# nianticlabs/implicit-depth

Measured on AMD Instinct MI355X. Metric: frames/sec (BDModel.forward hot path, 512x384, 64 planes, 8-frame tuple = 1 current + 7 source views; third-party backbones excluded), higher is better.
Workload: dtype f32

## Files before the change

### implicit-depth_amd/csrc/feature_volume.hip

```cpp
#include <stdlib.h>

#include "idh_common.h"
#include "split_f16.h"

namespace {

using namespace idh_f16;

constexpr int kC = 16;
constexpr int kHid = 128;
constexpr int kNS = 8;
constexpr int kMaxK = 8;

constexpr int kWsHom = 0, kWsT = 192, kWsInvK = 256, kWsBias = 272;
static_assert(kWsT == 12 * IDH_MAX_SOURCE_VIEWS && kWsInvK == kWsT + 4 * IDH_MAX_SOURCE_VIEWS && kWsBias + kHid <= 400, "workspace layout");
constexpr int kWsStrideReal = 400;

__device__ __forceinline__ float lrelu01(float x) {
#ifdef IDH_ABL_FV2_NOACT
    return x;
#endif
    return __builtin_elementwise_maximum(x, x * 0.01f);
}
__device__ __forceinline__ float lrelu01_sel(float x) { return x >= 0.f ? x : x * 0.01f; }

__device__ __forceinline__ float fv_depth_plane(int i, int D, float dmin, float dmax) {
    float ramp = 0.f;
    if (D > 1) {
        const float step = 1.0f / (float)(D - 1);
        ramp = (i < D / 2) ? step * (float)i : 1.0f - step * (float)(D - 1 - i);
    }
    return expf(logf(dmin) + logf(dmax / dmin) * ramp);
}

__global__ void fv_setup_k(const float *__restrict__ src_K, const float *__restrict__ src_E,
                           const float *__restrict__ src_poses, const float *__restrict__ cur_invK,
                           const float *__restrict__ w1_pose, const float *__restrict__ b1, int K,
                           float *__restrict__ ws) {
    const int b = blockIdx.x, t = threadIdx.x;
    float *o = ws + (size_t)b * kWsStrideReal;
    __shared__ float s_pd[3 * IDH_MAX_SOURCE_VIEWS];
    if (t < K) {
        const float *Km = src_K + (size_t)(b * K + t) * 16, *Em = src_E + (size_t)(b * K + t) * 16;
        const float *iK = cur_invK + (size_t)b * 16, *Pm = src_poses + (size_t)(b * K + t) * 16;
        float P[3][4];
        for (int i = 0; i < 3; ++i)
            for (int j = 0; j < 4; ++j) {
                float s = 0.f;
                for (int m = 0; m < 4; ++m) s = fmaf(Km[i * 4 + m], Em[m * 4 + j], s);
                P[i][j] = s;
            }
        float *h = o + kWsHom + 12 * t;
        for (int i = 0; i < 3; ++i) {
            for (int j = 0; j < 3; ++j) {
                float s = 0.f;
                for (int m = 0; m < 3; ++m) s = fmaf(P[i][m], iK[m * 4 + j], s);
                h[i * 3 + j] = s;
            }
            h[9 + i] = P[i][3];
        }
        o[kWsT + 4 * t + 0] = Pm[3]; o[kWsT + 4 * t + 1] = Pm[7]; o[kWsT + 4 * t + 2] = Pm[11]; o[kWsT + 4 * t + 3] = 0.f;
        const float tr = Pm[0] + Pm[5] + Pm[10];
        const float rm = sqrtf(2.f * (1.f - fminf(3.f, tr) / 3.f));
        const float tm = sqrtf(Pm[3] * Pm[3] + Pm[7] * Pm[7] + Pm[11] * Pm[11]);
        s_pd[t] = sqrtf(tm * tm + rm * rm);
        s_pd[K + t] = rm;
        s_pd[2 * K + t] = tm;
    }
    if (t < 9) o[kWsInvK + t] = cur_invK[(size_t)b * 16 + (t / 3) * 4 + (t % 3)];
    __syncthreads();
    if (t < kHid) {
        float s = b1[t];
        for (int j = 0; j < 3 * K; ++j) s = fmaf(w1_pose[(size_t)t * 3 * K + j], s_pd[j], s);
        o[kWsBias + t] = s;
    }
}

struct FvArgs {
    const float *cur;
    const float *src;
    const float *ws;
    const float *w1v;
    const float *w1p;
    const float *w2;
    const float *vecs;
    float *vol;
    unsigned char *mask;
    int vol_cs;
    int B, K, H, W, D;
    int tiles_per_img;
    int DP, G;
    int J, MB;
    float dmin, dmax;
    long long cur_bs, src_bs;
    const float *planes;
    long long planes_sb, planes_sd;
    int planes_sp;
};

__device__ __forceinline__ float fv_plane(const FvArgs &a, int b, int p, int d) {
    return a.planes ? a.planes[(size_t)b * a.planes_sb + (size_t)d * a.planes_sd + (size_t)p * a.planes_sp]
                    : fv_depth_plane(d, a.D, a.dmin, a.dmax);
}

template <int KT>
__global__ __launch_bounds__(512) void fv_mlp_k(const FvArgs a) {
    extern __shared__ __attribute__((aligned(16))) unsigned char smem_raw[];
    f32x4 *sW1 = reinterpret_cast<f32x4 *>(smem_raw);
    f32x4 *sW2 = sW1 + (a.K + 4) * kNS * 64;
    {
        const f32x4 *g1 = reinterpret_cast<const f32x4 *>(a.w1v);
        const f32x4 *g2 = reinterpret_cast<const f32x4 *>(a.w2);
        const int n1 = (a.K + 4) * kNS * 64, n2 = kNS * kNS * 64;
        for (int i = threadIdx.x; i < n1; i += 512) sW1[i] = g1[i];
        for (int i = threadIdx.x; i < n2; i += 512) sW2[i] = g2[i];
    }
    __syncthreads();
    const float *s_b2 = a.vecs, *s_w3 = a.vecs + kHid;
    const float b3 = a.vecs[2 * kHid];

    const int lane = threadIdx.x & 63;
    const int wave = __builtin_amdgcn_readfirstlane(threadIdx.x >> 6);
    const int ln = lane & 15, q = lane >> 4;
    const int N = a.H * a.W;
    const int K = KT > 0 ? KT : a.K;
    const float Wf = (float)a.W, Hf = (float)a.H;
    const long long ntasks = (long long)a.B * a.tiles_per_img * a.G;

    for (long long task = (long long)idh_xcd_remap(blockIdx.x, gridDim.x) * 8 + wave; task < ntasks; task += (long long)gridDim.x * 8) {
        const int g = __builtin_amdgcn_readfirstlane((int)(task % a.G));
        const int tile = __builtin_amdgcn_readfirstlane((int)((task / a.G) % a.tiles_per_img));
        const int b = __builtin_amdgcn_readfirstlane((int)(task / ((long long)a.G * a.tiles_per_img)));
        const int p_raw = tile * 16 + ln;
        const bool live = p_raw < N;
        const int p = live ? p_raw : N - 1;
        const int py = p / a.W, px = p - py * a.W;
        const float pxf = (float)px + 0.5f, pyf = (float)py + 0.5f;
        const float *pb = a.ws + (size_t)b * kWsStrideReal;

        const f32x4 cur4 = *reinterpret_cast<const f32x4 *>(a.cur + (size_t)b * a.cur_bs + (size_t)p * kC + 4 * q);
        const float *iK = pb + kWsInvK;
        const float rx = fmaf(iK[0], pxf, fmaf(iK[1], pyf, iK[2]));
        const float ry = fmaf(iK[3], pxf, fmaf(iK[4], pyf, iK[5]));
        const float rz = fmaf(iK[6], pxf, fmaf(iK[7], pyf, iK[8]));

        f32x4 pre[kNS];
#pragma unroll
        for (int i = 0; i < kNS; ++i) pre[i] = *reinterpret_cast<const f32x4 *>(pb + kWsBias + 16 * i + 4 * q);
        const int d0 = g * a.DP, d1 = min(a.D, d0 + a.DP);
        if (d0 >= d1) continue;
        const float rn = fmaxf(sqrtf(rx * rx + ry * ry + rz * rz), 1e-12f);
        const float crx = rx / rn, cry = ry / rn, crz = rz / rn;
        {
            const f32x4 rayB = (q == 0) ? (f32x4){crx, cry, crz, 0.f} : (f32x4){0.f, 0.f, 0.f, 0.f};
            const f32x4 *w1p = reinterpret_cast<const f32x4 *>(a.w1p);
#pragma unroll
            for (int i = 0; i < kNS; ++i) {
                const f32x4 A0 = w1p[(0 * kNS + i) * 64 + lane];
                const f32x4 A1 = w1p[(1 * kNS + i) * 64 + lane];
#pragma unroll
                for (int kk = 0; kk < 4; ++kk) pre[i] = __builtin_amdgcn_mfma_f32_16x16x4f32(A0[kk], cur4[kk], pre[i], 0, 0, 0);
#pragma unroll
                for (int kk = 0; kk < 4; ++kk) pre[i] = __builtin_amdgcn_mfma_f32_16x16x4f32(A1[kk], rayB[kk], pre[i], 0, 0, 0);
            }
        }

        const int ov[2] = {min(q, K - 1), min(q + 4, K - 1)};
        float oq[2][3], oh[2][3];
#pragma unroll
        for (int jv = 0; jv < 2; ++jv) {
            const float *hm = pb + kWsHom + 12 * ov[jv];
            oq[jv][0] = fmaf(hm[0], pxf, fmaf(hm[1], pyf, hm[2]));
            oq[jv][1] = fmaf(hm[3], pxf, fmaf(hm[4], pyf, hm[5]));
            oq[jv][2] = fmaf(hm[6], pxf, fmaf(hm[7], pyf, hm[8]));
            oh[jv][0] = hm[9]; oh[jv][1] = hm[10]; oh[jv][2] = hm[11];
        }
        const __amdgpu_buffer_rsrc_t rsS = __builtin_amdgcn_make_buffer_rsrc(const_cast<float *>(a.src + (size_t)b * a.src_bs), 0, K * N * kC * 4, 0x00020000);
        const int bp0 = 4 * ln;

        f32x4 ob = (f32x4){0.f, 0.f, 0.f, 0.f};
        const bool vec_ok = ((d0 & 3) == 0) && ((a.vol_cs & 3) == 0) && ((reinterpret_cast<uintptr_t>(a.vol) & 15) == 0);
        struct Own { int pk; float w00, w01, w10, w11, z; };
        struct Pro { Own own[2]; float depth, m3, m4, m5, m6, m10, m11, m12, m13; };
        struct Tap { f32x4 t00, t01, t10, t11; };
        struct Wts { float w00, w01, w10, w11; };
        float oc[2][3];
#pragma unroll
        for (int jv = 0; jv < 2; ++jv) {
            const float *t = pb + kWsT + 4 * ov[jv];
            oc[jv][0] = t[0]; oc[jv][1] = t[1]; oc[jv][2] = t[2];
        }
        auto prologue = [&](int d) {
            Pro P;
            const float depth = fv_plane(a, b, p, d);
            P.depth = depth;
#pragma unroll
            for (int jv = 0; jv < 2; ++jv) {
#ifdef IDH_ABL_FV2_NOPRO
                P.own[jv].pk = p; P.own[jv].w00 = P.own[jv].w01 = P.own[jv].w10 = P.own[jv].w11 = depth; P.own[jv].z = depth;
                continue;
#endif
                const float cx = fmaf(depth, oq[jv][0], oh[jv][0]);
                const float cy = fmaf(depth, oq[jv][1], oh[jv][1]);
                const float cz = fmaf(depth, oq[jv][2], oh[jv][2]);
                const float z = fmaxf(cz, 1e-5f);
                float r = __builtin_amdgcn_rcpf(z);
                r = r * fmaf(-z, r, 2.0f);
                const float su = cx * r, sv = cy * r;
                const float sx = fminf(fmaxf(su - 0.5f, -1.0f), Wf);
                const float sy = fminf(fmaxf(sv - 0.5f, -1.0f), Hf);
                const float x0f = floorf(sx), y0f = floorf(sy);
                const float fx = sx - x0f, fy = sy - y0f;
                const int x0 = (int)x0f, y0 = (int)y0f;
                const float wx0 = (x0 >= 0 && x0 < a.W) ? 1.0f - fx : 0.f;
                const float wx1 = (x0 + 1 < a.W) ? fx : 0.f;
                const float wy0 = (y0 >= 0 && y0 < a.H) ? 1.0f - fy : 0.f;
                const float wy1 = (y0 + 1 < a.H) ? fy : 0.f;
                const int xa0 = min(max(x0, 0), a.W - 1), xa1 = min(x0 + 1, a.W - 1);
                const int ya0 = min(max(y0, 0), a.H - 1), ya1 = min(y0 + 1, a.H - 1);
                P.own[jv].pk = (ya0 * a.W + xa0) | ((xa1 - xa0) << 30) | ((ya1 - ya0) << 31);
                P.own[jv].w00 = wx0 * wy0; P.own[jv].w01 = wx1 * wy0; P.own[jv].w10 = wx0 * wy1; P.own[jv].w11 = wx1 * wy1;
                P.own[jv].z = z;
            }
            const float Xx = depth * rx, Xy = depth * ry, Xz = depth * rz;
            auto ray = [&](int jv, float &ang, float &e0, float &e1, float &e2) {
                const float ax = Xx - oc[jv][0], ay = Xy - oc[jv][1], az = Xz - oc[jv][2];
                const float n2 = fmaf(az, az, fmaf(ay, ay, ax * ax));
                float in = __builtin_amdgcn_rsqf(fmaxf(n2, 1e-24f));
                in = in * fmaf(-0.5f * n2 * in, in, 1.5f);
                e0 = ax * in; e1 = ay * in; e2 = az * in;
                ang = fmaf(crz, e2, fmaf(cry, e1, crx * e0));
            };
#ifdef IDH_ABL_FV2_NORAY
            P.m3 = P.m4 = P.m5 = P.m6 = P.m10 = P.m11 = P.m12 = P.m13 = depth;
            return P;
#endif
            ray(0, P.m3, P.m4, P.m5, P.m6);
            ray(1, P.m10, P.m11, P.m12, P.m13);
            return P;
        };
        auto issue = [&](const Pro &P, int k) {
            const int pk = __builtin_amdgcn_ds_bpermute(bp0 + 64 * (k & 3), P.own[k >> 2].pk);
            const int o00 = ((pk & 0x3fffffff) << 6) + 16 * q;
            const int o01 = o00 + (((pk >> 30) & 1) << 6);
            const int ystep = (int)((unsigned)pk >> 31) * (a.W * 64);
            Tap t;
#ifdef IDH_ABL_FV2_NOTAPS
            t.t00 = t.t01 = t.t10 = t.t11 = (f32x4){1.f + (float)o00, 2.f + (float)o01, 3.f + (float)ystep, 4.f};
            return t;
#endif
            const int so = __builtin_amdgcn_readfirstlane(k * N * (kC * 4));
            t.t00 = __builtin_bit_cast(f32x4, __builtin_amdgcn_raw_buffer_load_b128(rsS, o00, so, 0));
            t.t01 = __builtin_bit_cast(f32x4, __builtin_amdgcn_raw_buffer_load_b128(rsS, o01, so, 0));
            t.t10 = __builtin_bit_cast(f32x4, __builtin_amdgcn_raw_buffer_load_b128(rsS, o00 + ystep, so, 0));
            t.t11 = __builtin_bit_cast(f32x4, __builtin_amdgcn_raw_buffer_load_b128(rsS, o01 + ystep, so, 0));
            return t;
        };
        auto weights = [&](const Pro &P, int k) {
            const Own &o = P.own[k >> 2];
            auto bperm = [&](float v) -> float { return __builtin_bit_cast(float, __builtin_amdgcn_ds_bpermute(bp0 + 64 * (k & 3), __builtin_bit_cast(int, v))); };
            Wts w;
            w.w00 = bperm(o.w00); w.w01 = bperm(o.w01); w.w10 = bperm(o.w10); w.w11 = bperm(o.w11);
            return w;
        };
        Pro P = prologue(d0);
        Tap cur = issue(P, 0);
        Wts wc = weights(P, 0);
#pragma unroll 1
        for (int d = d0; d < d1; ++d) {
            const float depth = P.depth;
            f32x4 acc1[kNS];
#pragma unroll
            for (int i = 0; i < kNS; ++i) acc1[i] = pre[i];
            float m2 = 0.f, m9 = 0.f;
            const float m1 = q < K ? P.own[0].z : 0.f;
            float m8 = q + 4 < K ? P.own[1].z : 0.f;
            __builtin_amdgcn_s_setprio(2);
            constexpr int KU = KT > 0 ? KT : kMaxK;
#pragma unroll
            for (int k = 0; k < KU; ++k) {
                if (KT == 0 && k >= K) break;
                const int kn = (KT > 0) ? (k + 1 < KT ? k + 1 : k) : k + 1;
                Tap nxt = cur;
                Wts wn = wc;
                if (kn != k && kn < KU) { nxt = issue(P, kn); wn = weights(P, kn); }
                f32x4 wv;
#ifdef IDH_ABL_FV2_NOBLEND
                wv = cur.t00 + cur.t11;
                float part = wc.w00 + wc.w11 + cur.t01[0] + cur.t10[0];
#else
#pragma unroll
                for (int e = 0; e < 4; ++e)
                    wv[e] = fmaf(wc.w11, cur.t11[e], fmaf(wc.w10, cur.t10[e], fmaf(wc.w01, cur.t01[e], wc.w00 * cur.t00[e])));
                float part = wv[0] * cur4[0];
                part = fmaf(wv[1], cur4[1], part); part = fmaf(wv[2], cur4[2], part); part = fmaf(wv[3], cur4[3], part);
                part += __shfl_xor(part, 16, 64);
                part += __shfl_xor(part, 32, 64);
#endif
                const float dotv = part;
                const bool s0 = (k == q), s1 = (k == q + 4);
                m2 = s0 ? dotv : m2;
                m9 = s1 ? dotv : m9;
#pragma unroll
                for (int i = 0; i < kNS; ++i) {
#ifdef IDH_ABL_FV2_NOLDSA
                    const f32x4 A = (f32x4){1.f, 2.f, 3.f, 4.f} * (float)(i + 1);
#else
                    const f32x4 A = sW1[(k * kNS + i) * 64 + lane];
#endif
#pragma unroll
                    for (int kk = 0; kk < 4; ++kk) acc1[i] = __builtin_amdgcn_mfma_f32_16x16x4f32(A[kk], wv[kk], acc1[i], 0, 0, 0);
                }
                if constexpr (KT > 0) {
#pragma unroll
                    for (int r = 0; r < 16; ++r) {
                        __builtin_amdgcn_sched_group_barrier(0x008, 2, 0);
#ifndef IDH_ABL_FV_VALU_PER_GROUP
#define IDH_ABL_FV_VALU_PER_GROUP 3
#endif
                        __builtin_amdgcn_sched_group_barrier(0x002, IDH_ABL_FV_VALU_PER_GROUP, 0);
                    }
                }
                cur = nxt;
                wc = wn;
            }
            const float m3 = P.m3, m4 = P.m4, m5 = P.m5, m6 = P.m6, m10 = P.m10, m11 = P.m11, m12 = P.m12, m13 = P.m13;
            const bool depth_in_q3 = K < 8;
            if (depth_in_q3 && q == 3) m8 = depth;
            const f32x4 mb[4] = {(f32x4){m1, m2, m3, m4}, (f32x4){m5, m6, m8, m9}, (f32x4){m10, m11, m12, m13}, (f32x4){depth, 0.f, 0.f, 0.f}};
#pragma unroll
            for (int c = 0; c < 3; ++c) {
#pragma unroll
                for (int i = 0; i < kNS; ++i) {
                    const f32x4 A = sW1[((K + c) * kNS + i) * 64 + lane];
#pragma unroll
                    for (int kk = 0; kk < 4; ++kk) acc1[i] = __builtin_amdgcn_mfma_f32_16x16x4f32(A[kk], mb[c][kk], acc1[i], 0, 0, 0);
                }
            }
            if (!depth_in_q3) {
#pragma unroll
                for (int i = 0; i < kNS; ++i) {
                    const float A0 = reinterpret_cast<const float *>(&sW1[((K + 3) * kNS + i) * 64 + lane])[0];
                    acc1[i] = __builtin_amdgcn_mfma_f32_16x16x4f32(A0, mb[3][0], acc1[i], 0, 0, 0);
                }
            }
            f32x4 acc2[kNS];
            Pro Pn;
            Tap curn;
            Wts wcn;
#pragma unroll
            for (int i = 0; i < kNS; ++i) {
#pragma unroll
                for (int r = 0; r < 4; ++r) acc1[i][r] = lrelu01(acc1[i][r]);
                acc2[i] = *reinterpret_cast<const f32x4 *>(s_b2 + 16 * i + 4 * q);
            }
            __builtin_amdgcn_s_setprio(0);
#pragma unroll
            for (int c = 0; c < kNS; ++c) {
#pragma unroll
                for (int i = 0; i < kNS; ++i) {
#ifdef IDH_ABL_FV2_NOLDSA
                    const f32x4 A = (f32x4){1.f, 2.f, 3.f, 4.f} * (float)(i + 1);
#else
                    const f32x4 A = sW2[(c * kNS + i) * 64 + lane];
#endif
#pragma unroll
                    for (int kk = 0; kk < 4; ++kk) acc2[i] = __builtin_amdgcn_mfma_f32_16x16x4f32(A[kk], acc1[c][kk], acc2[i], 0, 0, 0);
                }
                if (c == (KT > 0 ? 0 : 1)) {
                    Pn = prologue(min(d + 1, d1 - 1));
                    curn = issue(Pn, 0);
                    wcn = weights(Pn, 0);
                }
                if constexpr (KT == 0) __builtin_amdgcn_sched_barrier(0);
            }
            float s = 0.f;
#ifdef IDH_ABL_FV2_NOL3
#pragma unroll
            for (int i = 0; i < kNS; ++i) s += acc2[i][0];
#else
#pragma unroll
            for (int i = 0; i < kNS; ++i) {
                const f32x4 w3 = *reinterpret_cast<const f32x4 *>(s_w3 + 16 * i + 4 * q);
#pragma unroll
                for (int r = 0; r < 4; ++r) s = fmaf(w3[r], lrelu01(acc2[i][r]), s);
            }
            s += __shfl_xor(s, 16, 64);
            s += __shfl_xor(s, 32, 64);
#endif
            const float val = s + b3;
            if (a.vol_cs > 0) {
                const int e = (d - d0) & 3;
                ob[0] = e == 0 ? val : ob[0]; ob[1] = e == 1 ? val : ob[1]; ob[2] = e == 2 ? val : ob[2]; ob[3] = e == 3 ? val : ob[3];
                if (q == 0 && live && (e == 3 || d == d1 - 1)) {
                    float *o = a.vol + ((size_t)b * N + p) * a.vol_cs + (d - e);
                    if (e == 3 && vec_ok) *reinterpret_cast<f32x4 *>(o) = ob;
                    else { o[0] = ob[0]; if (e >= 1) o[1] = ob[1]; if (e >= 2) o[2] = ob[2]; if (e >= 3) o[3] = ob[3]; }
                }
            } else if (q == 0 && live) {
                a.vol[((size_t)b * a.D + d) * N + p] = val;
            }
            if (a.mask != nullptr && d == a.D - 1) {
                bool any_inb = false, any_front = false;
                for (int k = 0; k < K; ++k) {
                    const float *hm = pb + kWsHom + 12 * k;
                    const float qx = fmaf(hm[0], pxf, fmaf(hm[1], pyf, hm[2]));
                    const float qy = fmaf(hm[3], pxf, fmaf(hm[4], pyf, hm[5]));
                    const float qz = fmaf(hm[6], pxf, fmaf(hm[7], pyf, hm[8]));
                    const float cx = fmaf(depth, qx, hm[9]);
                    const float cy = fmaf(depth, qy, hm[10]);
                    const float cz = fmaf(depth, qz, hm[11]);
                    const float z = fmaxf(cz, 1e-5f);
                    float r = __builtin_amdgcn_rcpf(z);
                    r = r * fmaf(-z, r, 2.0f);
                    const float u = cx * r, v = cy * r;
                    any_inb |= (u > 2.f) & (u < Wf - 2.f) & (v > 2.f) & (v < Hf - 2.f);
                    any_front |= z > 0.f;
                }
                if (q == 0 && live) a.mask[(size_t)b * N + p] = (any_front && any_inb) ? 1 : 0;
            }
            P = Pn; cur = curn; wc = wcn;
        }
    }
}

template <int CB>
__global__ __launch_bounds__(512) void fv_mlp_gen_k(const FvArgs a) {
    extern __shared__ __attribute__((aligned(16))) unsigned char smem_raw[];
    f32x4 *sW2 = reinterpret_cast<f32x4 *>(smem_raw);
    {
        const f32x4 *g2 = reinterpret_cast<const f32x4 *>(a.w2);
        for (int i = threadIdx.x; i < kNS * kNS * 64; i += 512) sW2[i] = g2[i];
    }
    __syncthreads();
    const f32x4 *gW1 = reinterpret_cast<const f32x4 *>(a.w1v);
    const float *s_b2 = a.vecs, *s_w3 = a.vecs + kHid;
    const float b3 = a.vecs[2 * kHid];
    constexpr int kCc = kC * CB;

    const int lane = threadIdx.x & 63;
    const int wave = __builtin_amdgcn_readfirstlane(threadIdx.x >> 6);
    const int ln = lane & 15, q = lane >> 4;
    const int N = a.H * a.W;
    const int K = a.K, J = a.J;
    const float Wf = (float)a.W, Hf = (float)a.H;
    const long long ntasks = (long long)a.B * a.tiles_per_img * a.G;
    const int bp0 = 4 * ln;

    for (long long task = (long long)idh_xcd_remap(blockIdx.x, gridDim.x) * 8 + wave; task < ntasks; task += (long long)gridDim.x * 8) {
        const int g = __builtin_amdgcn_readfirstlane((int)(task % a.G));
        const int tile = __builtin_amdgcn_readfirstlane((int)((task / a.G) % a.tiles_per_img));
        const int b = __builtin_amdgcn_readfirstlane((int)(task / ((long long)a.G * a.tiles_per_img)));
        const int p_raw = tile * 16 + ln;
        const bool live = p_raw < N;
        const int p = live ? p_raw : N - 1;
        const int py = p / a.W, px = p - py * a.W;
        const float pxf = (float)px + 0.5f, pyf = (float)py + 0.5f;
        const float *pb = a.ws + (size_t)b * kWsStrideReal;

        f32x4 cur4[CB];
#pragma unroll
        for (int cb = 0; cb < CB; ++cb) cur4[cb] = *reinterpret_cast<const f32x4 *>(a.cur + (size_t)b * a.cur_bs + (size_t)p * kCc + 16 * cb + 4 * q);
        const float *iK = pb + kWsInvK;
        const float rx = fmaf(iK[0], pxf, fmaf(iK[1], pyf, iK[2]));
        const float ry = fmaf(iK[3], pxf, fmaf(iK[4], pyf, iK[5]));
        const float rz = fmaf(iK[6], pxf, fmaf(iK[7], pyf, iK[8]));

        f32x4 pre[kNS];
#pragma unroll
        for (int i = 0; i < kNS; ++i) pre[i] = *reinterpret_cast<const f32x4 *>(pb + kWsBias + 16 * i + 4 * q);
        const int d0 = g * a.DP, d1 = min(a.D, d0 + a.DP);
        if (d0 >= d1) continue;
        const float rn = fmaxf(sqrtf(rx * rx + ry * ry + rz * rz), 1e-12f);
        const float crx = rx / rn, cry = ry / rn, crz = rz / rn;
        {
            const f32x4 rayB = (q == 0) ? (f32x4){crx, cry, crz, 0.f} : (f32x4){0.f, 0.f, 0.f, 0.f};
            const f32x4 *w1p = reinterpret_cast<const f32x4 *>(a.w1p);
#pragma unroll
            for (int i = 0; i < kNS; ++i) {
#pragma unroll
                for (int cb = 0; cb < CB; ++cb) {
                    const f32x4 A0 = w1p[(cb * kNS + i) * 64 + lane];
#pragma unroll
                    for (int kk = 0; kk < 4; ++kk) pre[i] = __builtin_amdgcn_mfma_f32_16x16x4f32(A0[kk], cur4[cb][kk], pre[i], 0, 0, 0);
                }
                const f32x4 A1 = w1p[(CB * kNS + i) * 64 + lane];
#pragma unroll
                for (int kk = 0; kk < 4; ++kk) pre[i] = __builtin_amdgcn_mfma_f32_16x16x4f32(A1[kk], rayB[kk], pre[i], 0, 0, 0);
            }
        }
        const __amdgpu_buffer_rsrc_t rsS = __builtin_amdgcn_make_buffer_rsrc(const_cast<float *>(a.src + (size_t)b * a.src_bs), 0, K * N * kCc * 4, 0x00020000);

        f32x4 ob = (f32x4){0.f, 0.f, 0.f, 0.f};
        const bool vec_ok = ((d0 & 3) == 0) && ((a.vol_cs & 3) == 0) && ((reinterpret_cast<uintptr_t>(a.vol) & 15) == 0);
#pragma unroll 1
        for (int d = d0; d < d1; ++d) {
            const float depth = fv_plane(a, b, p, d);
            const float Xx = depth * rx, Xy = depth * ry, Xz = depth * rz;
            __builtin_amdgcn_s_setprio(2);
            f32x4 acc1[kNS];
#pragma unroll
            for (int i = 0; i < kNS; ++i) acc1[i] = pre[i];
            bool any_inb = false, any_front = false;
#pragma unroll 1
            for (int j = 0; j < J; ++j) {
                const int v = q + 4 * j, vs = min(v, K - 1);
                const bool mine = v < K;
                const float *hm = pb + kWsHom + 12 * vs;
                const float qx = fmaf(hm[0], pxf, fmaf(hm[1], pyf, hm[2]));
                const float qy = fmaf(hm[3], pxf, fmaf(hm[4], pyf, hm[5]));
                const float qz = fmaf(hm[6], pxf, fmaf(hm[7], pyf, hm[8]));
                const float cx = fmaf(depth, qx, hm[9]);
                const float cy = fmaf(depth, qy, hm[10]);
                const float cz = fmaf(depth, qz, hm[11]);
                const float z = fmaxf(cz, 1e-5f);
                float rc = __builtin_amdgcn_rcpf(z);
                rc = rc * fmaf(-z, rc, 2.0f);
                const float su = cx * rc, sv = cy * rc;
                any_inb |= mine & (su > 2.f) & (su < Wf - 2.f) & (sv > 2.f) & (sv < Hf - 2.f);
                any_front |= mine & (z > 0.f);
                const float sx = fminf(fmaxf(su - 0.5f, -1.0f), Wf);
                const float sy = fminf(fmaxf(sv - 0.5f, -1.0f), Hf);
                const float x0f = floorf(sx), y0f = floorf(sy);
                const float fx = sx - x0f, fy = sy - y0f;
                const int x0 = (int)x0f, y0 = (int)y0f;
                const float wx0 = (x0 >= 0 && x0 < a.W) ? 1.0f - fx : 0.f;
                const float wx1 = (x0 + 1 < a.W) ? fx : 0.f;
                const float wy0 = (y0 >= 0 && y0 < a.H) ? 1.0f - fy : 0.f;
                const float wy1 = (y0 + 1 < a.H) ? fy : 0.f;
                const int xa0 = min(max(x0, 0), a.W - 1), xa1 = min(x0 + 1, a.W - 1);
                const int ya0 = min(max(y0, 0), a.H - 1), ya1 = min(y0 + 1, a.H - 1);
                const int own_pk = (ya0 * a.W + xa0) | ((xa1 - xa0) << 30) | ((ya1 - ya0) << 31);
                const float own_w00 = wx0 * wy0, own_w01 = wx1 * wy0, own_w10 = wx0 * wy1, own_w11 = wx1 * wy1;
                float e0 = 0.f, e1 = 0.f, e2 = 0.f, ang = 0.f;
                {
                    const float *t = pb + kWsT + 4 * vs;
                    const float ax = Xx - t[0], ay = Xy - t[1], az = Xz - t[2];
                    const float in = 1.0f / fmaxf(sqrtf(ax * ax + ay * ay + az * az), 1e-12f);
                    e0 = ax * in; e1 = ay * in; e2 = az * in;
                    const float n1 = fmaxf(sqrtf(crx * crx + cry * cry + crz * crz), 1e-5f);
                    const float n2 = fmaxf(sqrtf(e0 * e0 + e1 * e1 + e2 * e2), 1e-5f);
                    ang = (crx * e0 + cry * e1 + crz * e2) / (n1 * n2);
                }
                const float maskv = z > 0.f ? 1.f : 0.f;
                float own_dot = 0.f;

                struct Tap { f32x4 t00[CB], t01[CB], t10[CB], t11[CB]; };
                struct Wts { float w00, w01, w10, w11; };
                auto issue = [&](int kq) {
                    const int pk = __builtin_amdgcn_ds_bpermute(bp0 + 64 * kq, own_pk);
                    const int o00 = (pk & 0x3fffffff) * (kCc * 4) + 16 * q;
                    const int o01 = o00 + ((pk >> 30) & 1) * (kCc * 4);
                    const int ystep = (int)((unsigned)pk >> 31) * (a.W * kCc * 4);
                    const int so = __builtin_amdgcn_readfirstlane((4 * j + kq) * N * (kCc * 4));
                    Tap t;
#pragma unroll
                    for (int cb = 0; cb < CB; ++cb) {
                        t.t00[cb] = __builtin_bit_cast(f32x4, __builtin_amdgcn_raw_buffer_load_b128(rsS, o00 + 64 * cb, so, 0));
                        t.t01[cb] = __builtin_bit_cast(f32x4, __builtin_amdgcn_raw_buffer_load_b128(rsS, o01 + 64 * cb, so, 0));
                        t.t10[cb] = __builtin_bit_cast(f32x4, __builtin_amdgcn_raw_buffer_load_b128(rsS, o00 + ystep + 64 * cb, so, 0));
                        t.t11[cb] = __builtin_bit_cast(f32x4, __builtin_amdgcn_raw_buffer_load_b128(rsS, o01 + ystep + 64 * cb, so, 0));
                    }
                    return t;
                };
                auto weights = [&](int kq) {
                    auto bperm = [&](float x) -> float { return __builtin_bit_cast(float, __builtin_amdgcn_ds_bpermute(bp0 + 64 * kq, __builtin_bit_cast(int, x))); };
                    Wts w;
                    w.w00 = bperm(own_w00); w.w01 = bperm(own_w01); w.w10 = bperm(own_w10); w.w11 = bperm(own_w11);
                    return w;
                };
                const int nv = min(4, K - 4 * j);
                Tap cur = issue(0);
                Wts wc = weights(0);
#pragma unroll
                for (int kq = 0; kq < 4; ++kq) {
                    if (kq >= nv) break;
                    Tap nxt = cur;
                    Wts wn = wc;
                    if (kq + 1 < 4 && kq + 1 < nv) { nxt = issue(kq + 1); wn = weights(kq + 1); }
                    float part = 0.f;
#pragma unroll
                    for (int cb = 0; cb < CB; ++cb) {
                        f32x4 wv;
#pragma unroll
                        for (int e = 0; e < 4; ++e)
                            wv[e] = fmaf(wc.w11, cur.t11[cb][e], fmaf(wc.w10, cur.t10[cb][e], fmaf(wc.w01, cur.t01[cb][e], wc.w00 * cur.t00[cb][e])));
                        float pc = wv[0] * cur4[cb][0];
                        pc = fmaf(wv[1], cur4[cb][1], pc); pc = fmaf(wv[2], cur4[cb][2], pc); pc = fmaf(wv[3], cur4[cb][3], pc);
                        part += pc;
#pragma unroll
                        for (int i = 0; i < kNS; ++i) {
                            const f32x4 A = gW1[((size_t)((4 * j + kq) * CB + cb) * kNS + i) * 64 + lane];
#pragma unroll
                            for (int kk = 0; kk < 4; ++kk) acc1[i] = __builtin_amdgcn_mfma_f32_16x16x4f32(A[kk], wv[kk], acc1[i], 0, 0, 0);
                        }
                    }
                    part += __shfl_xor(part, 16, 64);
                    part += __shfl_xor(part, 32, 64);
                    own_dot = (kq == q) ? part : own_dot;
                    cur = nxt;
                    wc = wn;
                }
                const f32x4 mb0 = mine ? (f32x4){maskv, z, own_dot * maskv, ang} : (f32x4){0.f, 0.f, 0.f, 0.f};
                const f32x4 mb1 = mine ? (f32x4){e0, e1, e2, (j == 0 && q == 0) ? depth : 0.f} : (f32x4){0.f, 0.f, 0.f, (j == 0 && q == 0) ? depth : 0.f};
#pragma unroll
                for (int c = 0; c < 2; ++c) {
#pragma unroll
                    for (int i = 0; i < kNS; ++i) {
                        const f32x4 A = gW1[((size_t)(K * CB + 2 * j + c) * kNS + i) * 64 + lane];
#pragma unroll
                        for (int kk = 0; kk < 4; ++kk) acc1[i] = __builtin_amdgcn_mfma_f32_16x16x4f32(A[kk], c == 0 ? mb0[kk] : mb1[kk], acc1[i], 0, 0, 0);
                    }
                }
            }
            f32x4 acc2[kNS];
#pragma unroll
            for (int i = 0; i < kNS; ++i) {
#pragma unroll
                for (int r = 0; r < 4; ++r) acc1[i][r] = lrelu01(acc1[i][r]);
                acc2[i] = *reinterpret_cast<const f32x4 *>(s_b2 + 16 * i + 4 * q);
            }
            __builtin_amdgcn_s_setprio(0);
#pragma unroll
            for (int c = 0; c < kNS; ++c) {
#pragma unroll
                for (int i = 0; i < kNS; ++i) {
                    const f32x4 A = sW2[(c * kNS + i) * 64 + lane];
#pragma unroll
                    for (int kk = 0; kk < 4; ++kk) acc2[i] = __builtin_amdgcn_mfma_f32_16x16x4f32(A[kk], acc1[c][kk], acc2[i], 0, 0, 0);
                }
                __builtin_amdgcn_sched_barrier(0);
            }
            float sacc = 0.f;
#pragma unroll
            for (int i = 0; i < kNS; ++i) {
                const f32x4 w3 = *reinterpret_cast<const f32x4 *>(s_w3 + 16 * i + 4 * q);
#pragma unroll
                for (int r = 0; r < 4; ++r) sacc = fmaf(w3[r], lrelu01(acc2[i][r]), sacc);
            }
            sacc += __shfl_xor(sacc, 16, 64);
            sacc += __shfl_xor(sacc, 32, 64);
            const float val = sacc + b3;
            if (a.vol_cs > 0) {
                const int e = (d - d0) & 3;
                ob[0] = e == 0 ? val : ob[0]; ob[1] = e == 1 ? val : ob[1]; ob[2] = e == 2 ? val : ob[2]; ob[3] = e == 3 ? val : ob[3];
                if (q == 0 && live && (e == 3 || d == d1 - 1)) {
                    float *o = a.vol + ((size_t)b * N + p) * a.vol_cs + (d - e);
                    if (e == 3 && vec_ok) *reinterpret_cast<f32x4 *>(o) = ob;
                    else { o[0] = ob[0]; if (e >= 1) o[1] = ob[1]; if (e >= 2) o[2] = ob[2]; if (e >= 3) o[3] = ob[3]; }
                }
            } else if (q == 0 && live) {
                a.vol[((size_t)b * a.D + d) * N + p] = val;
            }
            if (a.mask != nullptr && d == a.D - 1) {
                int fl = (any_inb ? 1 : 0) | (any_front ? 2 : 0);
                fl |= __shfl_xor(fl, 16, 64);
                fl |= __shfl_xor(fl, 32, 64);
                if (q == 0 && live) a.mask[(size_t)b * N + p] = (fl == 3) ? 1 : 0;
            }
        }
    }
}

template <int KT>
__global__ __launch_bounds__(512) void fv_mlp_f16_k(const FvArgs a, const float *__restrict__ sw1g, const float *__restrict__ sw2g) {
    extern __shared__ __attribute__((aligned(16))) unsigned char smem_raw[];
    const int K = KT > 0 ? KT : a.K;
    const int nb32 = (K + 5) / 2;
    u32x4 *sW1 = reinterpret_cast<u32x4 *>(smem_raw);
    u32x4 *sW2 = sW1 + nb32 * kNS * 2 * 64;
    {
        const u32x4 *g1 = reinterpret_cast<const u32x4 *>(a.w1v);
        const u32x4 *g2 = reinterpret_cast<const u32x4 *>(a.w2);
        const int n1 = nb32 * kNS * 2 * 64, n2 = 4 * kNS * 2 * 64;
        for (int i = threadIdx.x; i < n1; i += 512) sW1[i] = g1[i];
// ... 472 lines not shown
```

Before: 681.9.

## Skip source views with all-zero bilinear weights per plane and rotate task order

Computes a per-plane wave-wide mask of source views whose bilinear sampling weights are nonzero for some live pixel, and iterates only over those views with a dynamic ctz loop instead of a fully unrolled fixed-K loop. This avoids gathers and MFMA work for views whose projections fall entirely outside the image. It also rotates each wave's task index across grid strides to spread load. In exchange, the view loop is no longer unrolled at compile time, which may hurt instruction scheduling and register allocation. Skipping a view also leaves its contribution at zero, which should match the original since all of its weights were zero.

```diff
diff --git a/implicit-depth_amd/csrc/feature_volume.hip b/implicit-depth_amd/csrc/feature_volume.hip
--- a/implicit-depth_amd/csrc/feature_volume.hip
+++ b/implicit-depth_amd/csrc/feature_volume.hip
@@ -127,7 +127,15 @@
     const float Wf = (float)a.W, Hf = (float)a.H;
     const long long ntasks = (long long)a.B * a.tiles_per_img * a.G;
 
-    for (long long task = (long long)idh_xcd_remap(blockIdx.x, gridDim.x) * 8 + wave; task < ntasks; task += (long long)gridDim.x * 8) {
+#ifndef IDH_ABL_FV_TASK_ROT
+#define IDH_ABL_FV_TASK_ROT 5
+#endif
+    constexpr int kTaskRot = IDH_ABL_FV_TASK_ROT;
+    const long long S = (long long)gridDim.x * 8, first = (long long)idh_xcd_remap(blockIdx.x, gridDim.x) * 8 + wave;
+    long long rot = first;
+    for (long long base = 0; base < ntasks; base += S, rot = rot + kTaskRot >= S ? rot + kTaskRot - S : rot + kTaskRot) {
+        const long long task = base + (base + S <= ntasks ? rot : first);
+        if (task >= ntasks) break;
         const int g = __builtin_amdgcn_readfirstlane((int)(task % a.G));
         const int tile = __builtin_amdgcn_readfirstlane((int)((task / a.G) % a.tiles_per_img));
         const int b = __builtin_amdgcn_readfirstlane((int)(task / ((long long)a.G * a.tiles_per_img)));
@@ -181,7 +189,7 @@
         f32x4 ob = (f32x4){0.f, 0.f, 0.f, 0.f};
         const bool vec_ok = ((d0 & 3) == 0) && ((a.vol_cs & 3) == 0) && ((reinterpret_cast<uintptr_t>(a.vol) & 15) == 0);
         struct Own { int pk; float w00, w01, w10, w11, z; };
-        struct Pro { Own own[2]; float depth, m3, m4, m5, m6, m10, m11, m12, m13; };
+        struct Pro { Own own[2]; float depth, m3, m4, m5, m6, m10, m11, m12, m13; unsigned vm; };
         struct Tap { f32x4 t00, t01, t10, t11; };
         struct Wts { float w00, w01, w10, w11; };
         float oc[2][3];
@@ -192,6 +200,7 @@
         }
         auto prologue = [&](int d) {
             Pro P;
+            bool nz[2];
             const float depth = fv_plane(a, b, p, d);
             P.depth = depth;
 #pragma unroll
@@ -221,7 +230,24 @@
                 P.own[jv].pk = (ya0 * a.W + xa0) | ((xa1 - xa0) << 30) | ((ya1 - ya0) << 31);
                 P.own[jv].w00 = wx0 * wy0; P.own[jv].w01 = wx1 * wy0; P.own[jv].w10 = wx0 * wy1; P.own[jv].w11 = wx1 * wy1;
                 P.own[jv].z = z;
-            }
+                nz[jv] = live && (q + 4 * jv < K) &&
+                         ((__builtin_bit_cast(unsigned, P.own[jv].w00) | __builtin_bit_cast(unsigned, P.own[jv].w01) |
+                           __builtin_bit_cast(unsigned, P.own[jv].w10) | __builtin_bit_cast(unsigned, P.own[jv].w11)) != 0u);
+            }
+#if defined(IDH_ABL_FV_NOSKIP) || defined(IDH_ABL_FV2_NOPRO)
+            P.vm = (1u << K) - 1u;
+#else
+            {
+                const unsigned long long b0 = __ballot(nz[0]), b1 = __ballot(nz[1]);
+                unsigned vm = 0;
+#pragma unroll
+                for (int qq = 0; qq < 4; ++qq) {
+                    vm |= (((b0 >> (16 * qq)) & 0xffffull) != 0ull ? 1u : 0u) << qq;
+                    vm |= (((b1 >> (16 * qq)) & 0xffffull) != 0ull ? 1u : 0u) << (qq + 4);
+                }
+                P.vm = vm;
+            }
+#endif
             const float Xx = depth * rx, Xy = depth * ry, Xz = depth * rz;
             auto ray = [&](int jv, float &ang, float &e0, float &e1, float &e2) {
                 const float ax = Xx - oc[jv][0], ay = Xy - oc[jv][1], az = Xz - oc[jv][2];
@@ -240,7 +266,7 @@
             return P;
         };
         auto issue = [&](const Pro &P, int k) {
-            const int pk = __builtin_amdgcn_ds_bpermute(bp0 + 64 * (k & 3), P.own[k >> 2].pk);
+            const int pk = __builtin_amdgcn_ds_bpermute(bp0 + 64 * (k & 3), (k & 4) ? P.own[1].pk : P.own[0].pk);
             const int o00 = ((pk & 0x3fffffff) << 6) + 16 * q;
             const int o01 = o00 + (((pk >> 30) & 1) << 6);
             const int ystep = (int)((unsigned)pk >> 31) * (a.W * 64);
@@ -257,15 +283,17 @@
             return t;
         };
         auto weights = [&](const Pro &P, int k) {
-            const Own &o = P.own[k >> 2];
+            const bool hi = (k & 4) != 0;
             auto bperm = [&](float v) -> float { return __builtin_bit_cast(float, __builtin_amdgcn_ds_bpermute(bp0 + 64 * (k & 3), __builtin_bit_cast(int, v))); };
             Wts w;
-            w.w00 = bperm(o.w00); w.w01 = bperm(o.w01); w.w10 = bperm(o.w10); w.w11 = bperm(o.w11);
+            w.w00 = bperm(hi ? P.own[1].w00 : P.own[0].w00); w.w01 = bperm(hi ? P.own[1].w01 : P.own[0].w01);
+            w.w10 = bperm(hi ? P.own[1].w10 : P.own[0].w10); w.w11 = bperm(hi ? P.own[1].w11 : P.own[0].w11);
             return w;
         };
+        auto first_view = [](unsigned vm) { return vm ? __builtin_ctz(vm) : 0; };
         Pro P = prologue(d0);
-        Tap cur = issue(P, 0);
-        Wts wc = weights(P, 0);
+        Tap cur = issue(P, first_view(P.vm));
+        Wts wc = weights(P, first_view(P.vm));
 #pragma unroll 1
         for (int d = d0; d < d1; ++d) {
             const float depth = P.depth;
@@ -276,14 +304,14 @@
             const float m1 = q < K ? P.own[0].z : 0.f;
             float m8 = q + 4 < K ? P.own[1].z : 0.f;
             __builtin_amdgcn_s_setprio(2);
-            constexpr int KU = KT > 0 ? KT : kMaxK;
-#pragma unroll
-            for (int k = 0; k < KU; ++k) {
-                if (KT == 0 && k >= K) break;
-                const int kn = (KT > 0) ? (k + 1 < KT ? k + 1 : k) : k + 1;
-                Tap nxt = cur;
-                Wts wn = wc;
-                if (kn != k && kn < KU) { nxt = issue(P, kn); wn = weights(P, kn); }
+            unsigned vm = P.vm;
+#pragma unroll 1
+            while (vm) {
+                const int k = __builtin_ctz(vm);
+                vm &= vm - 1;
+                const int kn = vm ? __builtin_ctz(vm) : k;
+                const Tap nxt = issue(P, kn);
+                const Wts wn = weights(P, kn);
                 f32x4 wv;
 #ifdef IDH_ABL_FV2_NOBLEND
                 wv = cur.t00 + cur.t11;
@@ -301,25 +329,24 @@
                 const bool s0 = (k == q), s1 = (k == q + 4);
                 m2 = s0 ? dotv : m2;
                 m9 = s1 ? dotv : m9;
+                const f32x4 *sW1k = sW1 + k * (kNS * 64) + lane;
 #pragma unroll
                 for (int i = 0; i < kNS; ++i) {
 #ifdef IDH_ABL_FV2_NOLDSA
                     const f32x4 A = (f32x4){1.f, 2.f, 3.f, 4.f} * (float)(i + 1);
 #else
-                    const f32x4 A = sW1[(k * kNS + i) * 64 + lane];
+                    const f32x4 A = sW1k[i * 64];
 #endif
 #pragma unroll
                     for (int kk = 0; kk < 4; ++kk) acc1[i] = __builtin_amdgcn_mfma_f32_16x16x4f32(A[kk], wv[kk], acc1[i], 0, 0, 0);
                 }
-                if constexpr (KT > 0) {
-#pragma unroll
-                    for (int r = 0; r < 16; ++r) {
-                        __builtin_amdgcn_sched_group_barrier(0x008, 2, 0);
+#pragma unroll
+                for (int r = 0; r < 16; ++r) {
+                    __builtin_amdgcn_sched_group_barrier(0x008, 2, 0);
 #ifndef IDH_ABL_FV_VALU_PER_GROUP
 #define IDH_ABL_FV_VALU_PER_GROUP 3
 #endif
-                        __builtin_amdgcn_sched_group_barrier(0x002, IDH_ABL_FV_VALU_PER_GROUP, 0);
-                    }
+                    __builtin_amdgcn_sched_group_barrier(0x002, IDH_ABL_FV_VALU_PER_GROUP, 0);
                 }
                 cur = nxt;
                 wc = wn;
@@ -369,8 +396,8 @@
                 }
                 if (c == (KT > 0 ? 0 : 1)) {
                     Pn = prologue(min(d + 1, d1 - 1));
-                    curn = issue(Pn, 0);
-                    wcn = weights(Pn, 0);
+                    curn = issue(Pn, first_view(Pn.vm));
+                    wcn = weights(Pn, first_view(Pn.vm));
                 }
                 if constexpr (KT == 0) __builtin_amdgcn_sched_barrier(0);
             }
```

Measured after the change: 721.9, median of 6. 5.9% higher.
